# xissburg/edyn

Measured on AMD Instinct MI355X. Metric: steps/sec (whole node), 32k-box pile, 10 SI iters; HBM GB/s in solve, higher is better.
Workload: dtype f32

## Files before the change

edyn_amd/csrc/narrowphase.hip:

```cpp
#include "ctx.hpp"
#include "dpolyhedron.hpp"

namespace eh {
using namespace dc;

struct BodyIn { f3 pos; q4 orn; f3 angvel; float friction, restitution; bool rolling; };

DI f3 local_normal(const CPoint &rp, const BodyIn &A, const BodyIn &B) {
    return rp.attachment != NA_NONE ? rotate(conjugate(rp.attachment == NA_ON_A ? A.orn : B.orn), rp.normal) : mk3(0, 0, 0);
}
DI int find_nearest(const CPoint &cp, const CPoint (&rs)[4], int R) {
    float best = square(kCachingThreshold);
    int idx = R;
#pragma unroll
    for (int i = 0; i < 4; ++i) {
        if (i < R) {
            float dA = length_sqr(rs[i].pivotA - cp.pivotA);
            float dB = length_sqr(rs[i].pivotB - cp.pivotB);
            if (dA < best) { best = dA; idx = i; }
            if (dB < best) { best = dB; idx = i; }
        }
    }
    return idx;
}
DI int find_nearest_rolling(const CPoint (&rs)[4], int R, f3 cp_pivot, f3 origin, q4 orn, f3 angvel, float dt) {
    int idx = R;
    q4 prev_orn = integrate(orn, angvel, -dt);
    f3 prev_pivot = to_world(cp_pivot, origin, prev_orn);
    float best = square(kCachingThreshold);
#pragma unroll
    for (int i = 0; i < 4; ++i) {
        if (i < R) {
            f3 pA = to_world(rs[i].pivotA, origin, orn);
            float d2 = distance_sqr(pA, prev_pivot);
            if (d2 < best) { best = d2; idx = i; }
        }
    }
    return idx;
}
DI bool should_remove(const CPoint &cp, const BodyIn &A, const BodyIn &B) {
    const float thr = kBreakingThreshold, thr2 = thr * thr;
    f3 d = to_world(cp.pivotA, A.pos, A.orn) - to_world(cp.pivotB, B.pos, B.orn);
    float nd = dot(d, cp.normal);
    f3 td = d - nd * cp.normal;
    return nd > thr || length_sqr(td) > thr2;
}

struct Staging { float4 *ra, *rb, *rn; uint32_t *rnum; };

__global__ void __launch_bounds__(64, 2)
k_np_detect(uint32_t M, Manifolds mf, Bodies b, bool sleeping, Staging st) {
    const uint32_t m = blockIdx.x * blockDim.x + threadIdx.x;
    if (m >= M) return;
    const uint32_t ia = mf.bodyA[m], ib = mf.bodyB[m];
    const uint32_t fa = b.flags[ia], fb = b.flags[ib];
    if (sleeping && edge_asleep(fa, fb)) { st.rnum[m] = 0; return; }
    CResult res;
    res.num = 0;
    const box3 ba{from4(b.amin[ia]), from4(b.amax[ia])}, bbx{from4(b.amin[ib]), from4(b.amax[ib])};
    if (intersect(inset(ba, -kBreakingThreshold), bbx)) {
        const int tA = (int)((fa & BF_SHAPE_MASK) >> BF_SHAPE_SHIFT), tB = (int)((fb & BF_SHAPE_MASK) >> BF_SHAPE_SHIFT);
        Ctx ctx{B_ORG(b, ia), q_from4(B_ORN(b, ia)), B_ORG(b, ib), q_from4(B_ORN(b, ib)), kCollisionThreshold};
        collide(tA, b.shape[ia], tB, b.shape[ib], ctx, res);
    }
    st.rnum[m] = (uint32_t)res.num;
#pragma unroll
    for (int k = 0; k < kMaxPts; ++k) {
        if (k >= res.num) break;
        const size_t d = (size_t)k * mf.cap + m;
        st.ra[d] = to4(res.pt[k].pivotA, res.pt[k].distance);
        st.rb[d] = to4(res.pt[k].pivotB, __int_as_float(res.pt[k].attachment));
        st.rn[d] = to4(res.pt[k].normal, 0.0f);
    }
}

__global__ void __launch_bounds__(64)
k_np_detect_ext(uint32_t M, Manifolds mf, Bodies b, bool sleeping, Staging st) {
    const uint32_t m = blockIdx.x * blockDim.x + threadIdx.x;
    if (m >= M) return;
    const uint32_t ia = mf.bodyA[m], ib = mf.bodyB[m];
    const uint32_t fa = b.flags[ia], fb = b.flags[ib];
    const int tA = (int)((fa & BF_SHAPE_MASK) >> BF_SHAPE_SHIFT), tB = (int)((fb & BF_SHAPE_MASK) >> BF_SHAPE_SHIFT);
    if (tA != SHAPE_CYLINDER && tB != SHAPE_CYLINDER) return;
    if (sleeping && edge_asleep(fa, fb)) return;
    const box3 ba{from4(b.amin[ia]), from4(b.amax[ia])}, bbx{from4(b.amin[ib]), from4(b.amax[ib])};
    if (!intersect(inset(ba, -kBreakingThreshold), bbx)) return;
    CResult res;
    res.num = 0;
    Ctx ctx{B_ORG(b, ia), q_from4(B_ORN(b, ia)), B_ORG(b, ib), q_from4(B_ORN(b, ib)), kCollisionThreshold};
    collide_ext(tA, b.shape[ia], tB, b.shape[ib], ctx, res);
    st.rnum[m] = (uint32_t)res.num;
    for (int k = 0; k < res.num; ++k) {
        const size_t d = (size_t)k * mf.cap + m;
        st.ra[d] = to4(res.pt[k].pivotA, res.pt[k].distance);
        st.rb[d] = to4(res.pt[k].pivotB, __int_as_float(res.pt[k].attachment));
        st.rn[d] = to4(res.pt[k].normal, 0.0f);
    }
}

constexpr uint32_t kPolyBins = 1024;
constexpr uint32_t kPolyPairBins = 24 * 24;
struct PolyBins { uint32_t *count, *start, *cursor, *total, *key, *list, *hint; };
DI uint32_t poly_bin(int tA, float4 sA, int tB, float4 sB) {
    const uint32_t cA = (uint32_t)sA.x % 24u, cB = (uint32_t)sB.x % 24u;
    if (tA == SHAPE_POLYHEDRON && tB == SHAPE_POLYHEDRON) return cA * 24u + cB;
    return tA == SHAPE_POLYHEDRON ? kPolyPairBins + cA * 8u + ((uint32_t)tB & 7u) : kPolyPairBins + 192u + cB * 8u + ((uint32_t)tA & 7u);
}
__global__ void __launch_bounds__(256) k_poly_count(uint32_t M, Manifolds mf, Bodies b, bool sleeping, PolyBins pb, Meshes meshes, const uint32_t *hint_prev, bool rebuilt, bool use_hints) {
    __shared__ uint32_t hist[kPolyBins];
    for (uint32_t k = threadIdx.x; k < kPolyBins; k += 256) hist[k] = 0;
    __syncthreads();
    const uint32_t m = blockIdx.x * 256 + threadIdx.x;
    uint32_t key = 0xFFFFFFFFu;
    if (m < M) {
        const uint32_t ia = mf.bodyA[m], ib = mf.bodyB[m];
        const uint32_t fa = b.flags[ia], fb = b.flags[ib];
        const int tA = (int)((fa & BF_SHAPE_MASK) >> BF_SHAPE_SHIFT), tB = (int)((fb & BF_SHAPE_MASK) >> BF_SHAPE_SHIFT);
        if ((tA == SHAPE_POLYHEDRON || tB == SHAPE_POLYHEDRON) && !(sleeping && edge_asleep(fa, fb))) {
            const box3 ba{from4(b.amin[ia]), from4(b.amax[ia])}, bbx{from4(b.amin[ib]), from4(b.amax[ib])};
            if (intersect(inset(ba, -kBreakingThreshold), bbx)) key = poly_bin(tA, b.shape[ia], tB, b.shape[ib]);
        }
        uint32_t hint = 0;
        if (rebuilt) { const uint32_t p = mf.prev_idx[m]; if (p < mf.cap) hint = hint_prev[p]; } else hint = pb.hint[m];
        pb.hint[m] = hint;
        if (use_hints && hint != 0 && key < kPolyPairBins &&
            pp_hint_separates(meshes, pp_side(meshes, b.shape[ia], meshes.rot + meshes.rot_off[ia]), pp_side(meshes, b.shape[ib], meshes.rot + meshes.rot_off[ib]),
                              B_ORG(b, ib) - B_ORG(b, ia), kCollisionThreshold, hint)) key = 0xFFFFFFFFu;
        pb.key[m] = key;
    }
    if (key != 0xFFFFFFFFu) atomicAdd(&hist[key], 1u);
    __syncthreads();
    for (uint32_t k = threadIdx.x; k < kPolyBins; k += 256) if (hist[k]) atomicAdd(&pb.count[k], hist[k]);
}
__global__ void __launch_bounds__(1024) k_poly_scan(PolyBins pb) {
    __shared__ uint32_t part[16];
    const uint32_t t = threadIdx.x, lane = t & 63u, wave = t >> 6;
    const uint32_t v = pb.count[t];
    uint32_t inc = v;
#pragma unroll
    for (int off = 1; off < 64; off <<= 1) { const uint32_t u = __shfl_up(inc, off); if ((int)lane >= off) inc += u; }
    if (lane == 63) part[wave] = inc;
    __syncthreads();
    uint32_t base = 0;
    for (uint32_t w = 0; w < wave; ++w) base += part[w];
    pb.start[t] = base + inc - v;
    pb.cursor[t] = 0;
    pb.count[t] = 0;
    if (t == 1023) *pb.total = base + inc;
}
__global__ void __launch_bounds__(256) k_poly_scatter(uint32_t M, PolyBins pb) {
    __shared__ uint32_t hist[kPolyBins];
    for (uint32_t k = threadIdx.x; k < kPolyBins; k += 256) hist[k] = 0;
    __syncthreads();
    const uint32_t m = blockIdx.x * 256 + threadIdx.x;
    const uint32_t key = m < M ? pb.key[m] : 0xFFFFFFFFu;
    uint32_t rank = 0;
    if (key != 0xFFFFFFFFu) rank = atomicAdd(&hist[key], 1u);
    __syncthreads();
    for (uint32_t k = threadIdx.x; k < kPolyBins; k += 256) if (hist[k]) hist[k] = pb.start[k] + atomicAdd(&pb.cursor[k], hist[k]);
    __syncthreads();
    if (key != 0xFFFFFFFFu) pb.list[hist[key] + rank] = m;
}
__global__ void __launch_bounds__(64, 2)
k_np_detect_poly(uint32_t M, Manifolds mf, Bodies b, Staging st, Meshes meshes, PolyBins pb, bool pp_elsewhere) {
    const uint32_t i = (pp_elsewhere ? pb.start[kPolyPairBins] : 0u) + blockIdx.x * blockDim.x + threadIdx.x;
    if (i >= M || i >= *pb.total) return;
    const uint32_t m = pb.list[i];
    const uint32_t ia = mf.bodyA[m], ib = mf.bodyB[m];
    const uint32_t fa = b.flags[ia], fb = b.flags[ib];
    const int tA = (int)((fa & BF_SHAPE_MASK) >> BF_SHAPE_SHIFT), tB = (int)((fb & BF_SHAPE_MASK) >> BF_SHAPE_SHIFT);
    CResult res;
    res.num = 0;
    Ctx ctx{B_ORG(b, ia), q_from4(B_ORN(b, ia)), B_ORG(b, ib), q_from4(B_ORN(b, ib)), kCollisionThreshold};
    collide_poly(meshes, tA, b.shape[ia], tA == SHAPE_POLYHEDRON ? meshes.rot + meshes.rot_off[ia] : nullptr, tB, b.shape[ib],
                 tB == SHAPE_POLYHEDRON ? meshes.rot + meshes.rot_off[ib] : nullptr, ctx, res);
    st.rnum[m] = (uint32_t)res.num;
    for (int k = 0; k < res.num; ++k) {
        const size_t d = (size_t)k * mf.cap + m;
        st.ra[d] = to4(res.pt[k].pivotA, res.pt[k].distance);
        st.rb[d] = to4(res.pt[k].pivotB, __int_as_float(res.pt[k].attachment));
        st.rn[d] = to4(res.pt[k].normal, 0.0f);
    }
}

DI PPSide pp_side_of(const Meshes &meshes, const Bodies &b, uint32_t body) { return pp_side(meshes, b.shape[body], meshes.rot + meshes.rot_off[body]); }
template <int G, bool PROF>
__global__ void __launch_bounds__(64)
k_np_pp_axes(Manifolds mf, Bodies b, Staging st, Meshes meshes, PolyBins pb, unsigned long long *prof_out) {
    constexpr uint32_t kGroups = 64u / G;
    const uint32_t g = threadIdx.x / G;
    const uint32_t n = pb.start[kPolyPairBins];
    PPProf<PROF> prof;
    if (PROF) for (int k = 0; k < 8; ++k) prof.t[k] = 0;
    uint32_t iters = 0;
    for (uint32_t i = blockIdx.x * kGroups + g; i < n; i += gridDim.x * kGroups) {
        prof.stamp(0);
        const uint32_t m = pb.list[i];
        const uint32_t ia = mf.bodyA[m], ib = mf.bodyB[m];
        PPSeparation sep;
        const bool touching = pp_group_axes<G>(meshes, pp_side_of(meshes, b, ia), pp_side_of(meshes, b, ib), B_ORG(b, ib) - B_ORG(b, ia), kCollisionThreshold, sep, prof);
        if (threadIdx.x % G == 0) {
            pb.hint[m] = sep.hint;
            if (touching) {
                pb.key[atomicAdd(&pb.cursor[kPolyBins - 1], 1u)] = m;
                st.ra[m] = to4(sep.axis, sep.distance);
                st.rb[m] = make_float4(sep.projectionA, sep.projectionB, 0.0f, 0.0f);
            } else {
                st.rnum[m] = 0;
            }
        }
        prof.stamp(3);
        ++iters;
    }
    if (PROF && threadIdx.x % G == 0) {
        atomicAdd(&prof_out[0], (unsigned long long)iters);
        for (int k = 1; k < 4; ++k) atomicAdd(&prof_out[k], (unsigned long long)(prof.t[k] - prof.t[k - 1]));
    }
}
template <int G, bool PROF>
__global__ void __launch_bounds__(64)
k_np_pp_contacts(Manifolds mf, Bodies b, Staging st, Meshes meshes, PolyBins pb, unsigned long long *prof_out) {
    constexpr uint32_t kGroups = 64u / G;
    __shared__ __align__(16) unsigned char lds_raw[kGroups * sizeof(PPLds)];
    const uint32_t g = threadIdx.x / G;
    PPLds &lds = reinterpret_cast<PPLds *>(lds_raw)[g];
    const uint32_t n = pb.cursor[kPolyBins - 1];
    PPProf<PROF> prof;
    if (PROF) for (int k = 0; k < 8; ++k) prof.t[k] = 0;
    uint32_t iters = 0;
    for (uint32_t i = blockIdx.x * kGroups + g; i < n; i += gridDim.x * kGroups) {
        prof.stamp(2);
        const uint32_t m = pb.key[i];
        const uint32_t ia = mf.bodyA[m], ib = mf.bodyB[m];
        const float4 r0 = st.ra[m], r1 = st.rb[m];
        const PPSeparation sep{from4(r0), r0.w, r1.x, r1.y};
        CResult res;
        res.num = 0;
        const Ctx ctx{B_ORG(b, ia), q_from4(B_ORN(b, ia)), B_ORG(b, ib), q_from4(B_ORN(b, ib)), kCollisionThreshold};
        pp_group_contacts<G>(pp_side_of(meshes, b, ia), pp_side_of(meshes, b, ib), ctx, sep, lds, res, prof);
        if (threadIdx.x % G == 0) {
            st.rnum[m] = (uint32_t)res.num;
            for (int k = 0; k < res.num; ++k) {
                const size_t d = (size_t)k * mf.cap + m;
                st.ra[d] = to4(res.pt[k].pivotA, res.pt[k].distance);
                st.rb[d] = to4(res.pt[k].pivotB, __int_as_float(res.pt[k].attachment));
                st.rn[d] = to4(res.pt[k].normal, 0.0f);
            }
        }
        pp_group_sync();
        prof.stamp(6);
        ++iters;
    }
    if (PROF && threadIdx.x % G == 0) {
        atomicAdd(&prof_out[4], (unsigned long long)iters);
        for (int k = 3; k < 7; ++k) atomicAdd(&prof_out[k + 2], (unsigned long long)(prof.t[k] - prof.t[k - 1]));
    }
}

__global__ void __launch_bounds__(64, 2)
k_np_merge(uint32_t M, Manifolds mf, Bodies b, float dt, bool sleeping, Manifolds old, bool points_in_old, Staging st, EventSink ev) {
    const uint32_t m = blockIdx.x * blockDim.x + threadIdx.x;
    if (m < M) {
        const uint32_t ia = mf.bodyA[m], ib = mf.bodyB[m];
        const uint32_t info = mf.info[m];
        const int n_old = (int)(info & 0xFF);
        const uint32_t fa = b.flags[ia], fb = b.flags[ib];
        const Manifolds &src = points_in_old ? old : mf;
        const uint32_t sidx = points_in_old ? mf.prev_idx[m] : m;
        if (sleeping && edge_asleep(fa, fb)) {
            if (points_in_old)
                for (int k = 0; k < n_old; ++k) {
                    const size_t ts = pt_at(src.cap, (uint32_t)k, sidx), td = pt_at(mf.cap, (uint32_t)k, m);
                    mf.pA[td] = src.pA[ts]; mf.pB[td] = src.pB[ts]; mf.nrm[td] = src.nrm[ts]; mf.lnrm[td] = src.lnrm[ts]; mf.imp[td] = src.imp[ts];
                    const size_t s = slot_at(src.cap, (uint32_t)k, sidx), d = slot_at(mf.cap, (uint32_t)k, m);
                    if (mf.pid) mf.pid[d] = src.pid[s];
                    if (mf.xmat) { mf.xmat[d] = src.xmat[s]; mf.ximp[d] = src.ximp[s]; }
                }
            return;
        }
        const int tA = (int)((fa & BF_SHAPE_MASK) >> BF_SHAPE_SHIFT), tB = (int)((fb & BF_SHAPE_MASK) >> BF_SHAPE_SHIFT);
        BodyIn A, B;
        { A.pos = B_ORG(b, ia); A.orn = q_from4(B_ORN(b, ia)); A.angvel = from4(b.angvel[ia]);
          float2 mt = b.mat[ia]; A.friction = mt.x; A.restitution = mt.y;
          A.rolling = (fa & BF_KIND_MASK) == EDYNHIP_KIND_DYNAMIC && (tA == SHAPE_SPHERE || tA == SHAPE_CAPSULE || tA == SHAPE_CYLINDER); }
        { B.pos = B_ORG(b, ib); B.orn = q_from4(B_ORN(b, ib)); B.angvel = from4(b.angvel[ib]);
          float2 mt = b.mat[ib]; B.friction = mt.x; B.restitution = mt.y;
          B.rolling = (fb & BF_KIND_MASK) == EDYNHIP_KIND_DYNAMIC && (tB == SHAPE_SPHERE || tB == SHAPE_CAPSULE || tB == SHAPE_CYLINDER); }

        CPoint pts[kMaxPts];
#pragma unroll
        for (int k = 0; k < kMaxPts; ++k) {
            if (k < n_old) {
                const size_t s = pt_at(src.cap, (uint32_t)k, sidx);
                const float4 a = src.pA[s], bb = src.pB[s], n = src.nrm[s];
                CPoint &p = pts[k];
                p.pivotA = from4(a); p.pivotB = from4(bb); p.normal = from4(n); p.attachment = __float_as_int(n.w);
                p.distance = dot(p.normal, to_world(p.pivotA, A.pos, A.orn) - to_world(p.pivotB, B.pos, B.orn));
            } else {
                pts[k] = CPoint{};
            }
        }

        const int R = (int)st.rnum[m];
        CPoint rs[kMaxPts];
#pragma unroll
        for (int k = 0; k < kMaxPts; ++k) {
            if (k < R) {
                const size_t d = (size_t)k * mf.cap + m;
                const float4 ra = st.ra[d], rb = st.rb[d], rn = st.rn[d];
                rs[k] = CPoint{from4(ra), from4(rb), from4(rn), ra.w, __float_as_int(rb.w)};
            } else {
                rs[k] = CPoint{};
            }
        }

        uint32_t merged = 0, dead = 0, changed = 0;
        int num_points = n_old;
#pragma unroll
        for (int i = 0; i < kMaxPts; ++i) {
            if (i < n_old) {
                CPoint &cp = pts[i];
                int nearest = find_nearest(cp, rs, R);
                if (nearest == R && A.rolling) nearest = find_nearest_rolling(rs, R, cp.pivotA, A.pos, A.orn, A.angvel, dt);
                if (nearest == R && B.rolling) nearest = find_nearest_rolling(rs, R, cp.pivotB, B.pos, B.orn, B.angvel, dt);
                if (nearest < R && !((merged >> nearest) & 1u)) { cp = pick4(rs, nearest); changed |= 1u << i; merged |= 1u << nearest; }
                else if (should_remove(cp, A, B)) { dead |= 1u << i; --num_points; }
            }
        }
        const uint32_t all_r = (1u << R) - 1u;

        CPoint lp[kMaxPts];
        uint32_t create = 0;
        if ((merged & all_r) != all_r) {
            int lold[kMaxPts] = {-1, -1, -1, -1};
            int ltype[kMaxPts] = {INS_NONE, INS_NONE, INS_NONE, INS_NONE};
#pragma unroll
            for (int i = 0; i < kMaxPts; ++i) lp[i] = CPoint{};
            if (num_points > 0) {
                int k = 0;
#pragma unroll
                for (int i = 0; i < kMaxPts; ++i) {
                    if (i < n_old && !((dead >> i) & 1u)) {
                        CPoint loc = pts[i];
                        loc.attachment = NA_NONE;
                        put4(lp, k, loc);
                        put4(lold, k, i);
                        ++k;
                    }
                }
            } else {
                num_points = 1;
                lp[0] = rs[0];
                ltype[0] = INS_APPEND;
                merged |= 1u;
            }
#pragma unroll
            for (int r = 0; r < kMaxPts; ++r) {
                if (r < R && !((merged >> r) & 1u)) {
                    const CPoint rp = rs[r];
                    f3 piv[kMaxPts];
#pragma unroll
                    for (int i = 0; i < kMaxPts; ++i) piv[i] = lp[i].pivotA;
                    int ir = insertion_point_index(piv, num_points, rp.pivotA);
                    if ((ir & 0xFF) == INS_NONE) {
#pragma unroll
                        for (int i = 0; i < kMaxPts; ++i) piv[i] = lp[i].pivotB;
                        ir = insertion_point_index(piv, num_points, rp.pivotB);
                    }
                    if ((ir & 0xFF) != INS_NONE) { put4(lp, ir >> 8, rp); put4(ltype, ir >> 8, ir & 0xFF); }
                }
            }
#pragma unroll
            for (int i = 0; i < kMaxPts; ++i) {
                if (i < num_points) {
                    const int ty = ltype[i], lo = lold[i];
                    if (ty == INS_APPEND || (ty == INS_SIMILAR && lo < 0)) create |= 1u << i;
                    else if (ty == INS_SIMILAR) {
#pragma unroll
                        for (int j = 0; j < kMaxPts; ++j) sel(pts[j], j == lo, lp[i]);
                        changed |= 1u << lo;
                    } else if (ty == INS_REPLACE) {
                        if (lo >= 0) dead |= 1u << lo;
                        create |= 1u << i;
                    }
                }
            }
        }
        float4 ext_l[kMaxPts], ext_i[kMaxPts];
        float ext_f[kMaxPts];
        uint64_t ext_id[kMaxPts] = {0, 0, 0, 0};
        if (mf.pid) {
#pragma unroll
            for (int i = 0; i < kMaxPts; ++i) {
                if (i < n_old) {
                    ext_id[i] = src.pid[(size_t)i * src.cap + sidx];
                    if ((dead >> i) & 1u) emit_event(ev, EDYNHIP_EVENT_POINT_DESTROYED, ia, ib, ext_id[i]);
                }
            }
        }
#pragma unroll
        for (int i = 0; i < kMaxPts; ++i) {
            if (i < n_old && !((dead >> i) & 1u)) {
                const size_t s = pt_at(src.cap, (uint32_t)i, sidx);
                ext_l[i] = src.lnrm[s]; ext_i[i] = src.imp[s]; ext_f[i] = src.pB[s].w;
            } else {
                ext_l[i] = ext_i[i] = make_float4(0, 0, 0, 0); ext_f[i] = 0;
            }
        }
        int n_out = 0;
        if (create) {
            float friction = sqrtf(A.friction * B.friction);
            float restitution = fminf(A.restitution, B.restitution);
            if (const float *e = mix_lookup(b, ia, ib)) { restitution = e[0]; friction = e[1]; }
#pragma unroll
            for (int i = kMaxPts - 1; i >= 0; --i) {
                if ((create >> i) & 1u) {
                    const CPoint &p = lp[i];
                    const size_t d = pt_at(mf.cap, (uint32_t)n_out, m);
                    mf.pA[d] = to4(p.pivotA, p.distance);
                    mf.pB[d] = to4(p.pivotB, friction);
                    mf.nrm[d] = to4(p.normal, __int_as_float(p.attachment));
                    mf.lnrm[d] = to4(local_normal(p, A, B), restitution);
                    mf.imp[d] = make_float4(0, 0, 0, __uint_as_float(0u));
                    if (mf.pid) {
                        const uint64_t id = ((uint64_t)(ev.step + 1u) << 32) | ((uint64_t)m << 2) | (uint64_t)i;
                        mf.pid[slot_at(mf.cap, (uint32_t)n_out, m)] = id;
                        emit_event(ev, EDYNHIP_EVENT_POINT_CREATED, ia, ib, id);
                    }
                    ++n_out;
                }
            }
        }
#pragma unroll
        for (int i = 0; i < kMaxPts; ++i) {
            if (i < n_old && !((dead >> i) & 1u)) {
                const CPoint &p = pts[i];
                const size_t d = pt_at(mf.cap, (uint32_t)n_out, m);
                const f3 ln = ((changed >> i) & 1u) ? local_normal(p, A, B) : from4(ext_l[i]);
                mf.pA[d] = to4(p.pivotA, p.distance);
                mf.pB[d] = to4(p.pivotB, ext_f[i]);
                mf.nrm[d] = to4(p.normal, __int_as_float(p.attachment));
                mf.lnrm[d] = to4(ln, ext_l[i].w);
                mf.imp[d] = make_float4(ext_i[i].x, ext_i[i].y, ext_i[i].z, __uint_as_float(__float_as_uint(ext_i[i].w) + 1u));
                if (mf.pid) mf.pid[slot_at(mf.cap, (uint32_t)n_out, m)] = ext_id[i];
                ++n_out;
            }
        }
        if (mf.xmat) {
            float4 xm[kMaxPts], xi[kMaxPts];
#pragma unroll
            for (int i = 0; i < kMaxPts; ++i) {
                if (i < n_old && !((dead >> i) & 1u)) { const size_t s = (size_t)i * src.cap + sidx; xm[i] = src.xmat[s]; xi[i] = src.ximp[s]; }
                else { xm[i] = xi[i] = make_float4(0, 0, 0, 0); }
            }
            const float4 ma = b.mat2[ia], mb = b.mat2[ib];
            float stiff = kLarge, damp = kLarge;
            if (ma.z < kLarge || mb.z < kLarge) { stiff = 1.0f / (1.0f / ma.z + 1.0f / mb.z); damp = 1.0f / (1.0f / ma.w + 1.0f / mb.w); }
            float4 fresh = make_float4(fmaxf(ma.y, mb.y), fmaxf(ma.x, mb.x), stiff, damp);
            if (const float *e = mix_lookup(b, ia, ib)) fresh = make_float4(e[3], e[2], e[4], e[5]);
            int slot = 0;
#pragma unroll
            for (int i = kMaxPts - 1; i >= 0; --i) if ((create >> i) & 1u) { const size_t d = (size_t)slot * mf.cap + m; mf.xmat[d] = fresh; mf.ximp[d] = make_float4(0, 0, 0, 0); ++slot; }
#pragma unroll
            for (int i = 0; i < kMaxPts; ++i) if (i < n_old && !((dead >> i) & 1u)) { const size_t d = (size_t)slot * mf.cap + m; mf.xmat[d] = xm[i]; mf.ximp[d] = xi[i]; ++slot; }
        }
        uint32_t colour = info >> 8;
        if (n_out == 0) colour = kNoColour;
        mf.info[m] = (uint32_t)n_out | (colour << 8);
    }
}

__global__ void k_count_points(uint32_t M, const uint32_t *__restrict__ info, Counters *cnt) {
    uint32_t m = blockIdx.x * blockDim.x + threadIdx.x;
    uint32_t pts = m < M ? (info[m] & 0xFF) : 0, act = pts ? 1u : 0u;
#pragma unroll
    for (int off = 32; off > 0; off >>= 1) { pts += __shfl_xor(pts, off); act += __shfl_xor(act, off); }
    if ((threadIdx.x & 63) == 0 && pts) { atomicAdd(&cnt->num_points, pts); atomicAdd(&cnt->num_active, act); }
}
int count_points(edynhip_ctx *c) {
    EH_HIP(c, hipMemsetAsync(&c->cnt->num_points, 0, 2 * sizeof(uint32_t), c->stream));
    const uint32_t M = c->num_manifolds;
    if (M) hipLaunchKernelGGL(k_count_points, dim3((M + 255) / 256), dim3(256), 0, c->stream, M, c->m[c->cur].info, c->cnt);
    EH_HIP(c, hipGetLastError());
    return EDYNHIP_OK;
}

template <bool EXT>
__global__ void __launch_bounds__(64, EXT ? 1 : 2) k_debug_collide(uint32_t n, const int32_t *__restrict__ st, const float4 *__restrict__ sp, const float *__restrict__ pos,
                                const float4 *__restrict__ orn, float threshold, float *out, uint32_t *count) {
    uint32_t i = blockIdx.x * blockDim.x + threadIdx.x;
    if (i >= n) return;
    Ctx ctx{mk3(pos[6 * i], pos[6 * i + 1], pos[6 * i + 2]), q_from4(orn[2 * i]), mk3(pos[6 * i + 3], pos[6 * i + 4], pos[6 * i + 5]),
            q_from4(orn[2 * i + 1]), threshold};
    CResult r;
    if (EXT) { r.num = 0; if (!collide_ext(st[2 * i], sp[2 * i], st[2 * i + 1], sp[2 * i + 1], ctx, r)) return; }
    else collide(st[2 * i], sp[2 * i], st[2 * i + 1], sp[2 * i + 1], ctx, r);
    count[i] = (uint32_t)r.num;
    for (int k = 0; k < r.num; ++k) {
        float *o = out + ((size_t)i * 4 + k) * 11;
        o[0] = r.pt[k].pivotA.x; o[1] = r.pt[k].pivotA.y; o[2] = r.pt[k].pivotA.z;
        o[3] = r.pt[k].pivotB.x; o[4] = r.pt[k].pivotB.y; o[5] = r.pt[k].pivotB.z;
        o[6] = r.pt[k].normal.x; o[7] = r.pt[k].normal.y; o[8] = r.pt[k].normal.z;
        o[9] = r.pt[k].distance; o[10] = (float)r.pt[k].attachment;
    }
}
__global__ void __launch_bounds__(64)
k_debug_collide_poly(uint32_t first, uint32_t n, const int32_t *__restrict__ st, const float4 *__restrict__ sp, const float *__restrict__ pos,
                     const float4 *__restrict__ orn, float threshold, float *out, uint32_t *count, Meshes meshes, float4 *scratch, uint32_t stride, int group) {
    const uint32_t i = first + blockIdx.x;
    if (blockIdx.x >= n) return;
    const int tA = st[2 * i], tB = st[2 * i + 1];
    if (tA != SHAPE_POLYHEDRON && tB != SHAPE_POLYHEDRON) return;
    float4 *rot[2] = {scratch + (size_t)(2 * blockIdx.x) * stride, scratch + (size_t)(2 * blockIdx.x + 1) * stride};
    for (int side = 0; side < 2; ++side) {
        if (st[2 * i + side] != SHAPE_POLYHEDRON) continue;
        const MeshDesc d = meshes.desc[(uint32_t)sp[2 * i + side].x];
        const q4 q = q_from4(orn[2 * i + side]) * q4{0, 0, 0, 1};
        for (uint32_t k = threadIdx.x; k < d.rot_size; k += 64) rotate_mesh_item(meshes, d, q, rot[side], k);
    }
    __syncthreads();
    Ctx ctx{mk3(pos[6 * i], pos[6 * i + 1], pos[6 * i + 2]), q_from4(orn[2 * i]), mk3(pos[6 * i + 3], pos[6 * i + 4], pos[6 * i + 5]),
            q_from4(orn[2 * i + 1]), threshold};
    CResult r;
    r.num = 0;
    if (group != 0 && tA == SHAPE_POLYHEDRON && tB == SHAPE_POLYHEDRON) {
        __shared__ __align__(16) unsigned char lds_raw[sizeof(PPLds)];
        PPLds &lds = *reinterpret_cast<PPLds *>(lds_raw);
        if ((int)threadIdx.x >= group) return;
        PPProf<false> noprof;
        const PPSide A = pp_side(meshes, sp[2 * i], rot[0]), B = pp_side(meshes, sp[2 * i + 1], rot[1]);
        PPSeparation sep;
        if (group == 16) { if (pp_group_axes<16>(meshes, A, B, ctx.posB - ctx.posA, ctx.threshold, sep, noprof)) pp_group_contacts<16>(A, B, ctx, sep, lds, r, noprof); }
        else if (group == 4) { if (pp_group_axes<4>(meshes, A, B, ctx.posB - ctx.posA, ctx.threshold, sep, noprof)) pp_group_contacts<4>(A, B, ctx, sep, lds, r, noprof); }
        else if (pp_group_axes<8>(meshes, A, B, ctx.posB - ctx.posA, ctx.threshold, sep, noprof)) pp_group_contacts<8>(A, B, ctx, sep, lds, r, noprof);
        if (threadIdx.x != 0) return;
    } else {
        if (threadIdx.x != 0) return;
        collide_poly(meshes, tA, sp[2 * i], rot[0], tB, sp[2 * i + 1], rot[1], ctx, r);
    }
    count[i] = (uint32_t)r.num;
    for (int k = 0; k < r.num; ++k) {
        float *o = out + ((size_t)i * 4 + k) * 11;
        o[0] = r.pt[k].pivotA.x; o[1] = r.pt[k].pivotA.y; o[2] = r.pt[k].pivotA.z;
        o[3] = r.pt[k].pivotB.x; o[4] = r.pt[k].pivotB.y; o[5] = r.pt[k].pivotB.z;
        o[6] = r.pt[k].normal.x; o[7] = r.pt[k].normal.y; o[8] = r.pt[k].normal.z;
        o[9] = r.pt[k].distance; o[10] = (float)r.pt[k].attachment;
    }
}
int debug_collide(edynhip_ctx *c, uint32_t n, const int32_t *st, const float *sp, const float *pos, const float *orn, float threshold,
                  float *out, uint32_t *count) {
    if (n == 0) return EDYNHIP_OK;
    const size_t b_st = (size_t)n * 8, b_sp = (size_t)n * 32, b_pos = (size_t)n * 24, b_orn = (size_t)n * 32, b_out = (size_t)n * 44 * 4, b_cnt = (size_t)n * 4;
    auto up16 = [](size_t x) { return (x + 15) & ~(size_t)15; };
    const size_t o_sp = up16(b_st), o_pos = o_sp + up16(b_sp), o_orn = o_pos + up16(b_pos), o_out = o_orn + up16(b_orn), o_cnt = o_out + up16(b_out);
    char *d = nullptr;
    EH_HIP(c, hipMalloc((void **)&d, o_cnt + up16(b_cnt)));
    hipStream_t s = c->stream;
    hipError_t e = hipMemcpyAsync(d, st, b_st, hipMemcpyHostToDevice, s);
    if (e == hipSuccess) e = hipMemcpyAsync(d + o_sp, sp, b_sp, hipMemcpyHostToDevice, s);
    if (e == hipSuccess) e = hipMemcpyAsync(d + o_pos, pos, b_pos, hipMemcpyHostToDevice, s);
    if (e == hipSuccess) e = hipMemcpyAsync(d + o_orn, orn, b_orn, hipMemcpyHostToDevice, s);
    if (e == hipSuccess) e = hipMemsetAsync(d + o_out, 0, b_out, s);
    if (e == hipSuccess) {
        hipLaunchKernelGGL(k_debug_collide<false>, dim3((n + 63) / 64), dim3(64), 0, s, n, (const int32_t *)d, (const float4 *)(d + o_sp), (const float *)(d + o_pos),
                           (const float4 *)(d + o_orn), threshold, (float *)(d + o_out), (uint32_t *)(d + o_cnt));
        bool any_cyl = false;
        for (uint32_t i = 0; i < 2 * n && !any_cyl; ++i) any_cyl = st[i] == EDYNHIP_SHAPE_CYLINDER;
        if (any_cyl)
            hipLaunchKernelGGL(k_debug_collide<true>, dim3((n + 63) / 64), dim3(64), 0, s, n, (const int32_t *)d, (const float4 *)(d + o_sp), (const float *)(d + o_pos),
                               (const float4 *)(d + o_orn), threshold, (float *)(d + o_out), (uint32_t *)(d + o_cnt));
        bool any_poly = false;
        for (uint32_t i = 0; i < 2 * n; ++i)
            if (st[i] == EDYNHIP_SHAPE_POLYHEDRON) {
                any_poly = true;
                const float id = sp[4 * i];
                if (!(id >= 0) || id >= (float)c->host_meshes.desc.size()) { (void)hipStreamSynchronize(s); (void)hipFree(d); return set_error(c, EDYNHIP_ERR_INVALID, "edynhip_debug_collide: unknown mesh id"); }
            }
        if (any_poly) {
            uint32_t stride = 0;
            for (const MeshDesc &md : c->host_meshes.desc) stride = std::max(stride, md.rot_size);
            const uint32_t chunk = 16384;
            const int group = getenv("EDYNHIP_POLY_GROUP") ? atoi(getenv("EDYNHIP_POLY_GROUP")) : 8;
            float4 *scratch = nullptr;
            e = hipMalloc((void **)&scratch, (size_t)chunk * 2 * stride * sizeof(float4));
            for (uint32_t first = 0; first < n && e == hipSuccess; first += chunk) {
                const uint32_t cnt = std::min(chunk, n - first);
                hipLaunchKernelGGL(k_debug_collide_poly, dim3(cnt), dim3(64), 0, s, first, cnt, (const int32_t *)d, (const float4 *)(d + o_sp), (const float *)(d + o_pos),
                                   (const float4 *)(d + o_orn), threshold, (float *)(d + o_out), (uint32_t *)(d + o_cnt), c->meshes, scratch, stride, group);
            }
            if (e == hipSuccess) e = hipStreamSynchronize(s);
            if (scratch) (void)hipFree(scratch);
        }
        if (e == hipSuccess) e = hipMemcpyAsync(out, d + o_out, b_out, hipMemcpyDeviceToHost, s);
    }
    if (e == hipSuccess) e = hipMemcpyAsync(count, d + o_cnt, b_cnt, hipMemcpyDeviceToHost, s);
    if (e == hipSuccess) e = hipStreamSynchronize(s);
    (void)hipFree(d);
    if (e != hipSuccess) return set_error(c, EDYNHIP_ERR_HIP, "edynhip_debug_collide", e);
    return EDYNHIP_OK;
}

int narrowphase(edynhip_ctx *c) {
    const uint32_t M = c->num_manifolds;
    if (M == 0) return EDYNHIP_OK;
    const Staging st{c->np_ra, c->np_rb, c->np_rn, c->np_rnum};
    hipLaunchKernelGGL(k_np_detect, dim3((M + 63) / 64), dim3(64), 0, c->stream, M, c->m[c->cur], c->b, c->sleeping, st);
    if (c->has_cylinder) hipLaunchKernelGGL(k_np_detect_ext, dim3((M + 63) / 64), dim3(64), 0, c->stream, M, c->m[c->cur], c->b, c->sleeping, st);
    if (c->has_polyhedron) {
        EH_TRY(update_rotated(c));
        uint32_t *pw = c->poly_work;
        const size_t cap = c->m[0].cap;
        uint32_t *const hints = pw + 3 * kPolyBins + 1 + 2 * cap;
        const PolyBins pb{pw, pw + kPolyBins, pw + 2 * kPolyBins, pw + 3 * kPolyBins, pw + 3 * kPolyBins + 1, pw + 3 * kPolyBins + 1 + cap, hints + (size_t)c->cur * cap};
        static const bool use_hints = !(getenv("EDYNHIP_POLY_HINT") && getenv("EDYNHIP_POLY_HINT")[0] == '0');
        hipLaunchKernelGGL(k_poly_count, dim3((M + 255) / 256), dim3(256), 0, c->stream, M, c->m[c->cur], c->b, c->sleeping, pb, c->meshes, hints + (size_t)(c->cur ^ 1) * cap,
                           !c->inplace_step, use_hints);
        hipLaunchKernelGGL(k_poly_scan, dim3(1), dim3(1024), 0, c->stream, pb);
        hipLaunchKernelGGL(k_poly_scatter, dim3((M + 255) / 256), dim3(256), 0, c->stream, M, pb);
        static const int group = getenv("EDYNHIP_POLY_GROUP") ? atoi(getenv("EDYNHIP_POLY_GROUP")) : 8;
        if (group != 0) {
            const uint32_t waves = 5120;
            static const int group2 = getenv("EDYNHIP_POLY_GROUP2") ? atoi(getenv("EDYNHIP_POLY_GROUP2")) : 4;
            static const bool prof = getenv("EDYNHIP_PP_PROF") != nullptr;
            unsigned long long *&prof_dev = c->pp_prof_dev;
            int &prof_calls = c->pp_prof_calls;
            if (prof && !prof_dev) { void *q = nullptr; EH_HIP(c, hipMalloc(&q, 128)); c->allocs.push_back(q); prof_dev = (unsigned long long *)q; EH_HIP(c, hipMemsetAsync(prof_dev, 0, 128, c->stream)); }
            const Manifolds &mfc = c->m[c->cur];
            unsigned long long *const pd = prof ? prof_dev : nullptr;
            if (prof) {
                if (group == 16) hipLaunchKernelGGL((k_np_pp_axes<16, true>), dim3(waves), dim3(64), 0, c->stream, mfc, c->b, st, c->meshes, pb, pd);
                else hipLaunchKernelGGL((k_np_pp_axes<8, true>), dim3(waves), dim3(64), 0, c->stream, mfc, c->b, st, c->meshes, pb, pd);
                if (group2 == 8) hipLaunchKernelGGL((k_np_pp_contacts<8, true>), dim3(waves), dim3(64), 0, c->stream, mfc, c->b, st, c->meshes, pb, pd);
                else hipLaunchKernelGGL((k_np_pp_contacts<4, true>), dim3(waves), dim3(64), 0, c->stream, mfc, c->b, st, c->meshes, pb, pd);
            } else {
                if (group == 16) hipLaunchKernelGGL((k_np_pp_axes<16, false>), dim3(waves), dim3(64), 0, c->stream, mfc, c->b, st, c->meshes, pb, pd);
                else hipLaunchKernelGGL((k_np_pp_axes<8, false>), dim3(waves), dim3(64), 0, c->stream, mfc, c->b, st, c->meshes, pb, pd);
                if (group2 == 8) hipLaunchKernelGGL((k_np_pp_contacts<8, false>), dim3(waves), dim3(64), 0, c->stream, mfc, c->b, st, c->meshes, pb, pd);
                else if (group2 == 16) hipLaunchKernelGGL((k_np_pp_contacts<16, false>), dim3(waves), dim3(64), 0, c->stream, mfc, c->b, st, c->meshes, pb, pd);
                else hipLaunchKernelGGL((k_np_pp_contacts<4, false>), dim3(waves), dim3(64), 0, c->stream, mfc, c->b, st, c->meshes, pb, pd);
            }
            if (prof && ++prof_calls % 100 == 0) {
                unsigned long long h[16];
                EH_HIP(c, hipMemcpyAsync(h, prof_dev, 128, hipMemcpyDeviceToHost, c->stream));
                EH_HIP(c, hipStreamSynchronize(c->stream));
                EH_HIP(c, hipMemsetAsync(prof_dev, 0, 128, c->stream));
                const double p = 100.0 * (double)std::max<unsigned long long>(h[0], 1), q = 100.0 * (double)std::max<unsigned long long>(h[4], 1);
                fprintf(stderr, "[pp prof, G=%d/%d] pairs/step %.0f, us per pair-iteration: setup+faces %.2f edges %.2f stores+wait %.2f; survivors/step %.0f: setup+polygons %.2f hulls %.2f contacts %.2f stores+wait %.2f\n",
                        group, group2, h[0] / 100.0, h[1] / p, h[2] / p, h[3] / p, h[4] / 100.0, h[5] / q, h[6] / q, h[7] / q, h[8] / q);
            }
        }
        hipLaunchKernelGGL(k_np_detect_poly, dim3((M + 63) / 64), dim3(64), 0, c->stream, M, c->m[c->cur], c->b, st, c->meshes, pb, group != 0);
    }
    hipLaunchKernelGGL(k_np_merge, dim3((M + 63) / 64), dim3(64), 0, c->stream, M, c->m[c->cur], c->b, c->cfg.fixed_dt, c->sleeping, c->m[c->cur ^ 1], c->points_in_prev, st, event_sink(c));
    c->points_in_prev = false;
    EH_HIP(c, hipGetLastError());
    return EDYNHIP_OK;
}

}
```

Baseline: 794.9.

## Fuse basic narrowphase detection into the manifold merge kernel

```diff
diff --git a/edyn_amd/csrc/narrowphase.hip b/edyn_amd/csrc/narrowphase.hip
--- a/edyn_amd/csrc/narrowphase.hip
+++ b/edyn_amd/csrc/narrowphase.hip
@@ -47,32 +47,6 @@
 }
 
 struct Staging { float4 *ra, *rb, *rn; uint32_t *rnum; };
-
-__global__ void __launch_bounds__(64, 2)
-k_np_detect(uint32_t M, Manifolds mf, Bodies b, bool sleeping, Staging st) {
-    const uint32_t m = blockIdx.x * blockDim.x + threadIdx.x;
-    if (m >= M) return;
-    const uint32_t ia = mf.bodyA[m], ib = mf.bodyB[m];
-    const uint32_t fa = b.flags[ia], fb = b.flags[ib];
-    if (sleeping && edge_asleep(fa, fb)) { st.rnum[m] = 0; return; }
-    CResult res;
-    res.num = 0;
-    const box3 ba{from4(b.amin[ia]), from4(b.amax[ia])}, bbx{from4(b.amin[ib]), from4(b.amax[ib])};
-    if (intersect(inset(ba, -kBreakingThreshold), bbx)) {
-        const int tA = (int)((fa & BF_SHAPE_MASK) >> BF_SHAPE_SHIFT), tB = (int)((fb & BF_SHAPE_MASK) >> BF_SHAPE_SHIFT);
-        Ctx ctx{B_ORG(b, ia), q_from4(B_ORN(b, ia)), B_ORG(b, ib), q_from4(B_ORN(b, ib)), kCollisionThreshold};
-        collide(tA, b.shape[ia], tB, b.shape[ib], ctx, res);
-    }
-    st.rnum[m] = (uint32_t)res.num;
-#pragma unroll
-    for (int k = 0; k < kMaxPts; ++k) {
-        if (k >= res.num) break;
-        const size_t d = (size_t)k * mf.cap + m;
-        st.ra[d] = to4(res.pt[k].pivotA, res.pt[k].distance);
-        st.rb[d] = to4(res.pt[k].pivotB, __int_as_float(res.pt[k].attachment));
-        st.rn[d] = to4(res.pt[k].normal, 0.0f);
-    }
-}
 
 __global__ void __launch_bounds__(64)
 k_np_detect_ext(uint32_t M, Manifolds mf, Bodies b, bool sleeping, Staging st) {
@@ -106,7 +80,8 @@
     if (tA == SHAPE_POLYHEDRON && tB == SHAPE_POLYHEDRON) return cA * 24u + cB;
     return tA == SHAPE_POLYHEDRON ? kPolyPairBins + cA * 8u + ((uint32_t)tB & 7u) : kPolyPairBins + 192u + cB * 8u + ((uint32_t)tA & 7u);
 }
-__global__ void __launch_bounds__(256) k_poly_count(uint32_t M, Manifolds mf, Bodies b, bool sleeping, PolyBins pb, Meshes meshes, const uint32_t *hint_prev, bool rebuilt, bool use_hints) {
+__global__ void __launch_bounds__(256) k_poly_count(uint32_t M, Manifolds mf, Bodies b, bool sleeping, PolyBins pb, Meshes meshes, const uint32_t *hint_prev, bool rebuilt, bool use_hints,
+                                                     uint32_t *rnum) {
     __shared__ uint32_t hist[kPolyBins];
     for (uint32_t k = threadIdx.x; k < kPolyBins; k += 256) hist[k] = 0;
     __syncthreads();
@@ -116,7 +91,8 @@
         const uint32_t ia = mf.bodyA[m], ib = mf.bodyB[m];
         const uint32_t fa = b.flags[ia], fb = b.flags[ib];
         const int tA = (int)((fa & BF_SHAPE_MASK) >> BF_SHAPE_SHIFT), tB = (int)((fb & BF_SHAPE_MASK) >> BF_SHAPE_SHIFT);
-        if ((tA == SHAPE_POLYHEDRON || tB == SHAPE_POLYHEDRON) && !(sleeping && edge_asleep(fa, fb))) {
+        const bool poly = tA == SHAPE_POLYHEDRON || tB == SHAPE_POLYHEDRON;
+        if (poly && !(sleeping && edge_asleep(fa, fb))) {
             const box3 ba{from4(b.amin[ia]), from4(b.amax[ia])}, bbx{from4(b.amin[ib]), from4(b.amax[ib])};
             if (intersect(inset(ba, -kBreakingThreshold), bbx)) key = poly_bin(tA, b.shape[ia], tB, b.shape[ib]);
         }
@@ -127,6 +103,7 @@
             pp_hint_separates(meshes, pp_side(meshes, b.shape[ia], meshes.rot + meshes.rot_off[ia]), pp_side(meshes, b.shape[ib], meshes.rot + meshes.rot_off[ib]),
                               B_ORG(b, ib) - B_ORG(b, ia), kCollisionThreshold, hint)) key = 0xFFFFFFFFu;
         pb.key[m] = key;
+        if (poly && key == 0xFFFFFFFFu) rnum[m] = 0;
     }
     if (key != 0xFFFFFFFFu) atomicAdd(&hist[key], 1u);
     __syncthreads();
@@ -258,7 +235,7 @@
 }
 
 __global__ void __launch_bounds__(64, 2)
-k_np_merge(uint32_t M, Manifolds mf, Bodies b, float dt, bool sleeping, Manifolds old, bool points_in_old, Staging st, EventSink ev) {
+k_np_collide(uint32_t M, Manifolds mf, Bodies b, float dt, bool sleeping, Manifolds old, bool points_in_old, Staging st, uint32_t staged_shapes, EventSink ev) {
     const uint32_t m = blockIdx.x * blockDim.x + threadIdx.x;
     if (m < M) {
         const uint32_t ia = mf.bodyA[m], ib = mf.bodyB[m];
@@ -280,10 +257,36 @@
         }
         const int tA = (int)((fa & BF_SHAPE_MASK) >> BF_SHAPE_SHIFT), tB = (int)((fb & BF_SHAPE_MASK) >> BF_SHAPE_SHIFT);
         BodyIn A, B;
-        { A.pos = B_ORG(b, ia); A.orn = q_from4(B_ORN(b, ia)); A.angvel = from4(b.angvel[ia]);
+        A.pos = B_ORG(b, ia); A.orn = q_from4(B_ORN(b, ia));
+        B.pos = B_ORG(b, ib); B.orn = q_from4(B_ORN(b, ib));
+
+        CResult res;
+        res.num = 0;
+#pragma unroll
+        for (int k = 0; k < kMaxPts; ++k) res.pt[k] = CPoint{};
+        const box3 ba{from4(b.amin[ia]), from4(b.amax[ia])}, bbx{from4(b.amin[ib]), from4(b.amax[ib])};
+        if (intersect(inset(ba, -kBreakingThreshold), bbx)) {
+            const uint32_t ext = ((1u << tA) | (1u << tB)) & ((1u << SHAPE_CYLINDER) | (1u << SHAPE_POLYHEDRON));
+            if (ext == 0) {
+                Ctx ctx{A.pos, A.orn, B.pos, B.orn, kCollisionThreshold};
+                collide(tA, b.shape[ia], tB, b.shape[ib], ctx, res);
+            } else if ((ext & (1u << SHAPE_POLYHEDRON)) ? (staged_shapes >> SHAPE_POLYHEDRON) & 1u : (staged_shapes >> SHAPE_CYLINDER) & 1u) {
+                res.num = (int)st.rnum[m];
+#pragma unroll
+                for (int k = 0; k < kMaxPts; ++k) {
+                    if (k < res.num) {
+                        const size_t d = (size_t)k * mf.cap + m;
+                        const float4 ra = st.ra[d], rb = st.rb[d], rn = st.rn[d];
+                        res.pt[k] = CPoint{from4(ra), from4(rb), from4(rn), ra.w, __float_as_int(rb.w)};
+                    }
+                }
+            }
+        }
+
+        { A.angvel = from4(b.angvel[ia]);
           float2 mt = b.mat[ia]; A.friction = mt.x; A.restitution = mt.y;
           A.rolling = (fa & BF_KIND_MASK) == EDYNHIP_KIND_DYNAMIC && (tA == SHAPE_SPHERE || tA == SHAPE_CAPSULE || tA == SHAPE_CYLINDER); }
-        { B.pos = B_ORG(b, ib); B.orn = q_from4(B_ORN(b, ib)); B.angvel = from4(b.angvel[ib]);
+        { B.angvel = from4(b.angvel[ib]);
           float2 mt = b.mat[ib]; B.friction = mt.x; B.restitution = mt.y;
           B.rolling = (fb & BF_KIND_MASK) == EDYNHIP_KIND_DYNAMIC && (tB == SHAPE_SPHERE || tB == SHAPE_CAPSULE || tB == SHAPE_CYLINDER); }
 
@@ -301,18 +304,10 @@
             }
         }
 
-        const int R = (int)st.rnum[m];
+        const int R = res.num;
         CPoint rs[kMaxPts];
 #pragma unroll
-        for (int k = 0; k < kMaxPts; ++k) {
-            if (k < R) {
-                const size_t d = (size_t)k * mf.cap + m;
-                const float4 ra = st.ra[d], rb = st.rb[d], rn = st.rn[d];
-                rs[k] = CPoint{from4(ra), from4(rb), from4(rn), ra.w, __float_as_int(rb.w)};
-            } else {
-                rs[k] = CPoint{};
-            }
-        }
+        for (int k = 0; k < kMaxPts; ++k) rs[k] = k < R ? res.pt[k] : CPoint{};
 
         uint32_t merged = 0, dead = 0, changed = 0;
         int num_points = n_old;
@@ -604,7 +599,6 @@
     const uint32_t M = c->num_manifolds;
     if (M == 0) return EDYNHIP_OK;
     const Staging st{c->np_ra, c->np_rb, c->np_rn, c->np_rnum};
-    hipLaunchKernelGGL(k_np_detect, dim3((M + 63) / 64), dim3(64), 0, c->stream, M, c->m[c->cur], c->b, c->sleeping, st);
     if (c->has_cylinder) hipLaunchKernelGGL(k_np_detect_ext, dim3((M + 63) / 64), dim3(64), 0, c->stream, M, c->m[c->cur], c->b, c->sleeping, st);
     if (c->has_polyhedron) {
         EH_TRY(update_rotated(c));
@@ -614,7 +608,7 @@
         const PolyBins pb{pw, pw + kPolyBins, pw + 2 * kPolyBins, pw + 3 * kPolyBins, pw + 3 * kPolyBins + 1, pw + 3 * kPolyBins + 1 + cap, hints + (size_t)c->cur * cap};
         static const bool use_hints = !(getenv("EDYNHIP_POLY_HINT") && getenv("EDYNHIP_POLY_HINT")[0] == '0');
         hipLaunchKernelGGL(k_poly_count, dim3((M + 255) / 256), dim3(256), 0, c->stream, M, c->m[c->cur], c->b, c->sleeping, pb, c->meshes, hints + (size_t)(c->cur ^ 1) * cap,
-                           !c->inplace_step, use_hints);
+                           !c->inplace_step, use_hints, st.rnum);
         hipLaunchKernelGGL(k_poly_scan, dim3(1), dim3(1024), 0, c->stream, pb);
         hipLaunchKernelGGL(k_poly_scatter, dim3((M + 255) / 256), dim3(256), 0, c->stream, M, pb);
         static const int group = getenv("EDYNHIP_POLY_GROUP") ? atoi(getenv("EDYNHIP_POLY_GROUP")) : 8;
@@ -651,7 +645,9 @@
         }
         hipLaunchKernelGGL(k_np_detect_poly, dim3((M + 63) / 64), dim3(64), 0, c->stream, M, c->m[c->cur], c->b, st, c->meshes, pb, group != 0);
     }
-    hipLaunchKernelGGL(k_np_merge, dim3((M + 63) / 64), dim3(64), 0, c->stream, M, c->m[c->cur], c->b, c->cfg.fixed_dt, c->sleeping, c->m[c->cur ^ 1], c->points_in_prev, st, event_sink(c));
+    const uint32_t staged_shapes = (c->has_cylinder ? 1u << SHAPE_CYLINDER : 0u) | (c->has_polyhedron ? 1u << SHAPE_POLYHEDRON : 0u);
+    hipLaunchKernelGGL(k_np_collide, dim3((M + 63) / 64), dim3(64), 0, c->stream, M, c->m[c->cur], c->b, c->cfg.fixed_dt, c->sleeping, c->m[c->cur ^ 1], c->points_in_prev, st,
+                       staged_shapes, event_sink(c));
     c->points_in_prev = false;
     EH_HIP(c, hipGetLastError());
     return EDYNHIP_OK;
```

Result: no change. 802.8 (median of 6 runs) (+1.0%).
